# vitskvara/VBMatrixFactorization.jl

Measured on AMD Instinct MI355X. Metric: VB iterations/sec, higher is better.
Workload: dtype bf16

## Files before the change

### vbmatrixfactorization.jl_amd/csrc/gram_kernels.hpp

```cpp
#pragma once
#include "common.hpp"
#include "ctrl_kernels.hpp"
#include "post_kernels.hpp"

namespace vbmf {

#ifndef GRAM_CHUNK
#define GRAM_CHUNK 256
#endif
constexpr int GRAM_PLANES = 5;

__device__ __forceinline__ unsigned pack_bf2(unsigned short lo, unsigned short hi) { return (unsigned)lo | ((unsigned)hi << 16); }

__global__ __launch_bounds__(256) void gram_build_kernel(const uint4* __restrict__ Y1, int XT, int KS, float* __restrict__ Gt,
                                                         int GT) {
    const int P = blockIdx.y, Q = blockIdx.x;
    if (P > Q) return;
    const int lane = threadIdx.x & 63, w = threadIdx.x >> 6;
    const int p0 = 4 * P + 2 * (w >> 1), q0 = 4 * Q + 2 * (w & 1);
    const long long KT = 2LL * GT;
    double g64[2][2][16];
#pragma unroll
    for (int a = 0; a < 2; ++a)
#pragma unroll
// ... 114 lines not shown
            Wnew[m * HP + h] = wv;
            wp[0][e] = f2bf(wv);
            float res = wv - bf2f(wp[0][e]);
            wp[1][e] = f2bf(res);
            res -= bf2f(wp[1][e]);
            wp[2][e] = f2bf(res);
            dp[0][e] = f2bf(dv);
            dp[1][e] = f2bf(dv - bf2f(dp[0][e]));
        }
        const long long o = (j * NH + ht) * 64 + ln;
#pragma unroll
        for (int p = 0; p < 3; ++p)
            Wt[p * plane + o] = make_uint4(pack_bf2(wp[p][0], wp[p][1]), pack_bf2(wp[p][2], wp[p][3]), pack_bf2(wp[p][4], wp[p][5]),
                                           pack_bf2(wp[p][6], wp[p][7]));
#pragma unroll
        for (int p = 0; p < 2; ++p)
            Wt[(3 + p) * plane + o] = make_uint4(pack_bf2(dp[p][0], dp[p][1]), pack_bf2(dp[p][2], dp[p][3]), pack_bf2(dp[p][4], dp[p][5]),
                                                 pack_bf2(dp[p][6], dp[p][7]));
    }
}

__device__ __forceinline__ float sub_f32(float a, float b) {
    float r;
    asm("v_sub_f32 %0, %1, %2" : "=v"(r) : "v"(a), "v"(b));
    return r;
}
__device__ __forceinline__ unsigned cvt_pk_bf16(float lo, float hi) {
    typedef __attribute__((ext_vector_type(2))) float f32x2v;
    typedef __attribute__((ext_vector_type(2))) __bf16 bf16x2v;
    const f32x2v v = {lo, hi};
    return __builtin_bit_cast(unsigned, __builtin_convertvector(v, bf16x2v));
}
__device__ __forceinline__ void split3_frag(const f32x4& x0, const f32x4& x1, u32x4v& g0, u32x4v& g1, u32x4v& g2) {
    const float v[8] = {x0.x, x0.y, x0.z, x0.w, x1.x, x1.y, x1.z, x1.w};
#pragma unroll
    for (int e = 0; e < 4; ++e) {
        float a = v[2 * e], b = v[2 * e + 1];
        const unsigned p0 = cvt_pk_bf16(a, b);
        a = sub_f32(a, bitsf(p0 << 16));
        b = sub_f32(b, bitsf(p0 & 0xffff0000u));
        const unsigned p1 = cvt_pk_bf16(a, b);
        a = sub_f32(a, bitsf(p1 << 16));
        b = sub_f32(b, bitsf(p1 & 0xffff0000u));
        g0[e] = p0;
        g1[e] = p1;
        g2[e] = cvt_pk_bf16(a, b);
    }
}

__device__ __forceinline__ f32x16 mfma_bf(const u32x4v& a, const u32x4v& b, const f32x16& c) {
    return __builtin_amdgcn_mfma_f32_32x32x16_bf16(__builtin_bit_cast(bf16x8, a), __builtin_bit_cast(bf16x8, b), c, 0, 0, 0);
}

template <int NH>
struct GramProd {
    static constexpr int NW = 8;
    static constexpr int THREADS = 64 * NW;
    static constexpr int TPG = 16 / NH;
    static constexpr int NXW = TPG >= NW ? TPG / NW : 1;
    static constexpr int HS = TPG >= NW ? 1 : NW / TPG;
    static constexpr int NHW = NH / HS;
    static constexpr int CH = NH == 2 ? 4 : 2;
    static constexpr int D = 4;
    static constexpr int U = CH;
    static constexpr int NP = GRAM_PLANES * CH * NH;
    static constexpr int PPW = (NP + NW - 1) / NW;
    static constexpr int GL = 2 * NXW;
    static constexpr int PLANE_BYTES = 2 * NP * 1024;
    static constexpr int RING_BYTES = NW * D * GL * 1024;
    static constexpr int LDS_BYTES = PLANE_BYTES + RING_BYTES;
    static_assert(NXW * (NW / HS) == TPG && NHW * HS == NH, "gram_prod geometry");
    static_assert(LDS_BYTES <= 160 * 1024, "gram_prod LDS");
    static constexpr int g_wait(int u) {
        int n = (D - 1) * GL;
        for (int d = 1; d < D; ++d) n += ((u + CH * D - d) % CH == 0) ? PPW : 0;
        return n;
    }
};
template <int NH>
__global__ __launch_bounds__(GramProd<NH>::THREADS) void gram_prod_kernel(const float4* __restrict__ Gt, const uint4* __restrict__ Wt,
                                                                          float* __restrict__ Out, int GT, int XT1, int sps, int nrg,
                                                                          long long n, long long slab_floats,
                                                                          const int* __restrict__ stop) {
    using C = GramProd<NH>;
    constexpr int NW = C::NW, NXW = C::NXW, NHW = C::NHW, D = C::D, CH = C::CH, U = C::U, NP = C::NP, PPW = C::PPW, GL = C::GL;
    extern __shared__ __attribute__((aligned(1024))) unsigned char gram_lds[];
    if (*stop) return;
    const int lane = threadIdx.x & 63;
    const int w = __builtin_amdgcn_readfirstlane(threadIdx.x >> 6);
    const int rg = blockIdx.x % nrg, s = blockIdx.x / nrg;
    const int KT = 2 * GT;
    const int j0 = s * sps, j1 = min(j0 + sps, KT), nk = j1 - j0;
    const int pt0 = rg * C::TPG + (w % (C::TPG / NXW)) * NXW;
    const int h0 = (w / (C::TPG / NXW)) * NHW;
    const long long plane = (long long)KT * NH * 64;
    f32x16 accP[NXW][NHW], accQ[NXW][NHW];
#pragma unroll
    for (int i = 0; i < NXW; ++i)
#pragma unroll
        for (int h = 0; h < NHW; ++h)
#pragma unroll
            for (int r = 0; r < 16; ++r) { accP[i][h][r] = 0.f; accQ[i][h][r] = 0.f; }
    __amdgpu_buffer_rsrc_t gr[NXW];
#pragma unroll
    for (int i = 0; i < NXW; ++i)
        gr[i] = __builtin_amdgcn_make_buffer_rsrc((void*)(Gt + (long long)(pt0 + i) * KT * 128), 0, (unsigned)KT * 2048u, 0x00020000);
    const __amdgpu_buffer_rsrc_t wr = __builtin_amdgcn_make_buffer_rsrc((void*)Wt, 0, (unsigned)(GRAM_PLANES * plane * 16), 0x00020000);
    const int voff = lane * 16;
    unsigned char* const ring = gram_lds + C::PLANE_BYTES + w * (D * GL * 1024);
    auto load_g = [&](int slot, int t) __attribute__((always_inline)) {
        const int so = min(j0 + t, j1 - 1) * 2048;
#pragma unroll
        for (int i = 0; i < NXW; ++i) {
            lds_dma_piece(gr[i], ring + (slot * GL + 2 * i) * 1024, voff, so);
            lds_dma_piece(gr[i], ring + (slot * GL + 2 * i + 1) * 1024, voff, so + 1024);
        }
    };
    auto load_planes = [&](int cc, int t) __attribute__((always_inline)) {
#pragma unroll
        for (int v = 0; v < PPW; ++v) {
            const int x = min(w + NW * v, NP - 1);
            const int q = x / (CH * NH), r = x % (CH * NH);
            const int j = min(j0 + t + r / NH, j1 - 1);
            lds_dma_piece(wr, gram_lds + (cc * NP + x) * 1024, voff, (int)(q * plane + ((long long)j * NH + r % NH) * 64) * 16);
        }
    };
#pragma unroll
    for (int d = 0; d < D; ++d) {
        if ((d + CH * D - D) % CH == 0) load_planes(0, 0);
        load_g(d, d);
    }
    asm volatile("s_waitcnt vmcnt(%0)" ::"n"(CH * GL) : "memory");
    __builtin_amdgcn_s_barrier();
    asm volatile("" ::: "memory");
    u32x4v wf[GRAM_PLANES][NHW], g[NXW][3];
    auto mma = [&]() __attribute__((always_inline)) {
#pragma unroll
        for (int i = 0; i < NXW; ++i) {
#pragma unroll
            for (int h = 0; h < NHW; ++h) {
                f32x16 a = accP[i][h];
                a = mfma_bf(wf[2][h], g[i][0], a);
                a = mfma_bf(wf[1][h], g[i][1], a);
                a = mfma_bf(wf[0][h], g[i][2], a);
                a = mfma_bf(wf[1][h], g[i][0], a);
                a = mfma_bf(wf[0][h], g[i][1], a);
                accP[i][h] = mfma_bf(wf[0][h], g[i][0], a);
                f32x16 d = accQ[i][h];
                d = mfma_bf(wf[4][h], g[i][0], d);
                d = mfma_bf(wf[3][h], g[i][1], d);
                accQ[i][h] = mfma_bf(wf[3][h], g[i][0], d);
            }
        }
    };
    int slot = 0;
    auto body = [&](int t0, bool tail) __attribute__((always_inline)) {
#pragma unroll
        for (int u = 0; u < U; ++u) {
            const int t = t0 + u, kk = u % CH;
            const int cc = (t / CH) & 1;
            const bool live = !tail || t < nk;
            asm volatile("s_waitcnt vmcnt(%0)" ::"n"(C::g_wait(u)) : "memory");
            if (live) {
                const unsigned char* gs = ring + slot * (GL * 1024) + lane * 32;
                f32x4 x[NXW][2];
#pragma unroll
                for (int i = 0; i < NXW; ++i) {
                    x[i][0] = *reinterpret_cast<const f32x4*>(gs + i * 2048);
                    x[i][1] = *reinterpret_cast<const f32x4*>(gs + i * 2048 + 16);
                }
                const unsigned char* pl = gram_lds + (cc * NP + kk * NH + h0) * 1024 + lane * 16;
#pragma unroll
                for (int q = 0; q < GRAM_PLANES; ++q)
#pragma unroll
                    for (int h = 0; h < NHW; ++h) wf[q][h] = *reinterpret_cast<const u32x4v*>(pl + (q * CH * NH + h) * 1024);
#pragma unroll
                for (int i = 0; i < NXW; ++i) split3_frag(x[i][0], x[i][1], g[i][0], g[i][1], g[i][2]);
            }
            __builtin_amdgcn_sched_barrier(0);
            if (kk == 0) load_planes(cc ^ 1, t + CH);
            load_g(slot, t + D);
            slot = slot + 1 == D ? 0 : slot + 1;
            __builtin_amdgcn_sched_barrier(0);
            if (live) mma();
            if (kk == CH - 1) {
                asm volatile("s_waitcnt vmcnt(%0) lgkmcnt(0)" ::"n"(CH * GL) : "memory");
                __builtin_amdgcn_s_barrier();
                asm volatile("" ::: "memory");
            }
        }
    };
    int t0 = 0;
    for (; t0 + U <= nk; t0 += U) body(t0, false);
    if (t0 < nk) body(t0, true);
    asm volatile("s_waitcnt vmcnt(0)" ::: "memory");
    float4* oP = reinterpret_cast<float4*>(Out + (long long)s * slab_floats);
    float4* oQ = reinterpret_cast<float4*>(Out + (long long)s * slab_floats + n);
#pragma unroll
    for (int i = 0; i < NXW; ++i) {
        const int p = pt0 + i;
        if (p >= XT1) continue;
#pragma unroll
        for (int h = 0; h < NHW; ++h) {
            const long long o = (((long long)p * NH + h0 + h) * 64 + lane) * 4;
            const f32x16 a = accP[i][h], d = accQ[i][h];
#pragma unroll
            for (int q = 0; q < 4; ++q) {
                oP[o + q] = float4{a[4 * q], a[4 * q + 1], a[4 * q + 2], a[4 * q + 3]};
                oQ[o + q] = float4{d[4 * q], d[4 * q + 1], d[4 * q + 2], d[4 * q + 3]};
            }
        }
    }
}

template <int HP>
struct GPart {
    static constexpr int V = HP / 16, S = 8 / V, NH = HP / 32;
};
template <int HP>
__device__ __forceinline__ int gpart_index(int a, int b) {
    constexpr int V = GPart<HP>::V;
    const int tw = a % V, i = a / V, t = b % V, c = b / V;
    return ((((tw * V + t) * 4 + (i >> 2)) << 6) + 16 * (i & 3) + c);
}
template <int HP>
__global__ __launch_bounds__(1024) void gram_part_kernel(const float* __restrict__ PQ, long long n, const float* __restrict__ Wn,
                                                         const float* __restrict__ Wo, const float* __restrict__ A32, long long M,
                                                         int rpc, double* __restrict__ part, const int* __restrict__ stop) {
    if (*stop) return;
    constexpr int V = GPart<HP>::V, S = GPart<HP>::S, NH = GPart<HP>::NH, U = 4;
    __shared__ f64x4 fold[S > 1 ? (S - 1) * 2 * V * V * 64 : 1];
    __shared__ double red[16];
    const int lane = threadIdx.x & 63, w = threadIdx.x >> 6;
    const int s = w / (2 * V), task = w % (2 * V), pi = task / V, tw = task % V;
    const int q = lane >> 4, c = lane & 15;
    const float* src = PQ + (pi ? n : 0);
    f64x4 acc[V];
#pragma unroll
    for (int t = 0; t < V; ++t) acc[t] = f64x4{0.0, 0.0, 0.0, 0.0};
    double tr = 0.0;
    const long long m0 = (long long)blockIdx.x * rpc, m1 = min(m0 + rpc, M);
    const int nstep = (int)((m1 - m0 + 3) / 4);
    for (int k0 = s; k0 < nstep; k0 += S * U) {
        float pv[U][V], wv[U], xv[U];
#pragma unroll
        for (int u = 0; u < U; ++u) {
            const long long m = m0 + 4LL * (k0 + u * S) + q;
            if (m < m1) {
                if constexpr (V == 2) {
                    const float2 v = *reinterpret_cast<const float2*>(src + frag_index(2 * c, m, NH));
                    pv[u][0] = v.x; pv[u][1] = v.y;
                } else {
#pragma unroll
                    for (int g = 0; g < V / 4; ++g) {
                        const float4 v = *reinterpret_cast<const float4*>(src + frag_index(V * c + 4 * g, m, NH));
                        pv[u][4 * g] = v.x; pv[u][4 * g + 1] = v.y; pv[u][4 * g + 2] = v.z; pv[u][4 * g + 3] = v.w;
                    }
                }
                wv[u] = Wn[m * HP + V * c + tw];
                xv[u] = (pi ? Wo : A32)[m * HP + V * c + tw];
            } else {
#pragma unroll
                for (int t = 0; t < V; ++t) pv[u][t] = 0.f;
                wv[u] = 0.f; xv[u] = 0.f;
            }
        }
#pragma unroll
        for (int u = 0; u < U; ++u) {
            double a = (double)wv[u];
            if (pi) a = (double)(float)(a - (double)xv[u]);
            else {
                float p = 0.f;
#pragma unroll
                for (int t = 0; t < V; ++t) p = t == tw ? pv[u][t] : p;
                tr += (double)xv[u] * (double)p;
            }
#pragma unroll
            for (int t = 0; t < V; ++t) acc[t] = __builtin_amdgcn_mfma_f64_16x16x4f64(a, (double)pv[u][t], acc[t], 0, 0, 0);
        }
    }
    if constexpr (S > 1) {
        if (s > 0) {
#pragma unroll
            for (int t = 0; t < V; ++t) fold[(((s - 1) * 2 * V + task) * V + t) * 64 + lane] = acc[t];
        }
        __syncthreads();
        if (s == 0) {
            for (int s2 = 1; s2 < S; ++s2)
#pragma unroll
                for (int t = 0; t < V; ++t) acc[t] += fold[(((s2 - 1) * 2 * V + task) * V + t) * 64 + lane];
        }
    }
    double* o = part + (long long)blockIdx.x * (2 * HP * HP + 1) + pi * HP * HP;
    if (s == 0) {
#pragma unroll
        for (int t = 0; t < V; ++t)
#pragma unroll
            for (int r = 0; r < 4; ++r) o[(((tw * V + t) * 4 + r) << 6) + lane] = acc[t][r];
    }
    tr = block_sum(tr, red);
    if (threadIdx.x == 0) part[(long long)blockIdx.x * (2 * HP * HP + 1) + 2 * HP * HP] = tr;
}

constexpr int GRED_E = 64, GRED_G = 4;
template <int HP>
__global__ __launch_bounds__(256) void gram_part_reduce_kernel(const double* __restrict__ part, int nchunk, double* __restrict__ st,
                                                               StateLayout lay, const int* __restrict__ stop) {
    if (*stop) return;
    constexpr int V = GPart<HP>::V, n2 = HP * HP;
    constexpr long long stride = 2LL * n2 + 1;
    __shared__ double sum[2][GRED_G][GRED_E];
    const int el = threadIdx.x % GRED_E, g = threadIdx.x / GRED_E;
    const int e = blockIdx.x * GRED_E + el;
    const int pi = e / n2, x = e % n2;
    const int tw = (x >> 8) / V, t = (x >> 8) % V, rq = (x >> 6) & 3, q = (x >> 4) & 3, c = x & 15;
    const int a = V * (q + 4 * rq) + tw, b = V * c + t;
    const bool mat = e < 2 * n2, tro = e == 2 * n2;
    const long long i0 = mat ? e : 2LL * n2, i1 = mat ? (long long)pi * n2 + gpart_index<HP>(b, a) : 2LL * n2;
    double s0 = 0.0, s1 = 0.0;
    if (mat || tro) {
        int k = g;
        for (; k + 7 * GRED_G < nchunk; k += 8 * GRED_G) {
            double v0[8], v1[8];
#pragma unroll
            for (int u = 0; u < 8; ++u) { v0[u] = part[(k + u * GRED_G) * stride + i0]; v1[u] = part[(k + u * GRED_G) * stride + i1]; }
#pragma unroll
            for (int u = 0; u < 8; ++u) { s0 += v0[u]; s1 += v1[u]; }
        }
        for (; k < nchunk; k += GRED_G) { s0 += part[k * stride + i0]; s1 += part[k * stride + i1]; }
    }
    sum[0][g][el] = s0;
    sum[1][g][el] = s1;
    __syncthreads();
    if (g != 0 || !(mat || tro)) return;
    double t0 = 0.0, t1 = 0.0;
    for (int k = 0; k < GRED_G; ++k) { t0 += sum[0][k][el]; t1 += sum[1][k][el]; }
    if (tro) st[lay.GX()] = t0;
    else st[(pi ? lay.GD() : lay.GB()) + a * HP + b] = 0.5 * (t0 + t1);
}

}
```

### vbmatrixfactorization.jl_amd/csrc/vbmf_hip.hip

```cpp
#include "../../include/vbmf_hip.h"

#include <hip/hip_runtime.h>
#include <rccl/rccl.h>

#include <algorithm>
#include <cmath>
#include <cstdio>
#include <cstring>
#include <string>
#include <vector>

#include "common.hpp"
#include "ctrl_kernels.hpp"
#include "post_kernels.hpp"
#include "rng.hpp"
#include "sparse_kernels.hpp"
#include "stream_gemm.hpp"
#include "tile_kernels.hpp"
#include "prep_kernels.hpp"
#include "batch_kernels.hpp"
#include "sparse_batch_kernels.hpp"
#include "score_kernels.hpp"
#include "gram_kernels.hpp"

// ... 880 lines not shown
        if (e != hipSuccess) {
            for (void* b : {(void*)c->Gt, (void*)c->W32g[0], (void*)c->W32g[1], (void*)c->Wt, (void*)c->gPQ, (void*)c->gslabs,
                            (void*)c->g_part, (void*)c->gsave})
                if (b) hipFree(b);
            c->Gt = nullptr; c->W32g[0] = c->W32g[1] = nullptr; c->Wt = nullptr; c->gPQ = nullptr; c->gslabs = nullptr;
            c->g_part = nullptr; c->gsave = nullptr;
            FAIL(c, VBMF_ERR_HIP, "Gram-form sweep: device allocation failed (%s)", hipGetErrorString(e));
        }
        c->G_valid = false;
    }
    if (c->G_valid) return VBMF_OK;
    hipEvent_t a, b;
    HIPCHK(c, hipEventCreate(&a));
    HIPCHK(c, hipEventCreate(&b));
    hipEventRecord(a, c->stream);
    const int NB = c->GT / 4;
    hipLaunchKernelGGL(gram_build_kernel, dim3(NB, NB), dim3(256), 0, c->stream, c->Y1, c->d1.XT, c->d1.KS, c->Gt, c->GT);
    const hipError_t le = hipGetLastError();
    hipEventRecord(b, c->stream);
    const hipError_t se = hipEventSynchronize(b);
    float ms = 0.f;
    hipEventElapsedTime(&ms, a, b);
    hipEventDestroy(a);
    hipEventDestroy(b);
    HIPCHK(c, le);
    HIPCHK(c, se);
    c->gram_build_ms = ms;
    c->G_valid = true;
    c->W_valid = false;
    return VBMF_OK;
}

static int gram_product(vbmf_ctx* c, bool partials) {
    const int* stop = c->ints + I_STOP;
    const int KT = 2 * c->GT;
    const int64_t Mp1 = (int64_t)c->d1.XT * 32;
    const long long n = (long long)c->Hp * Mp1;
    const float* Wo = c->W32g[c->wcur];
    float* Wn = c->W32g[c->wcur ^ 1];
    const dim3 wg(cdiv(KT, GW_KS));
    if (c->Hp == 32) hipLaunchKernelGGL((gram_w_kernel<32>), wg, dim3(128), 0, c->stream, c->A32, c->SB32, Wo, Wn, c->Wt, (long long)c->M, KT, stop);
    else if (c->Hp == 64) hipLaunchKernelGGL((gram_w_kernel<64>), wg, dim3(256), 0, c->stream, c->A32, c->SB32, Wo, Wn, c->Wt, (long long)c->M, KT, stop);
    else hipLaunchKernelGGL((gram_w_kernel<128>), wg, dim3(512), 0, c->stream, c->A32, c->SB32, Wo, Wn, c->Wt, (long long)c->M, KT, stop);
    HIPCHK(c, hipGetLastError());
    float* out = c->g_nsplit > 1 ? c->gslabs : c->gPQ;
    const dim3 grid(c->g_nrg * c->g_nsplit);
    const float4* G4 = reinterpret_cast<const float4*>(c->Gt);
    prof_begin(c, 0);
    if (c->NH == 1) hipLaunchKernelGGL((gram_prod_kernel<1>), grid, dim3(GramProd<1>::THREADS), GramProd<1>::LDS_BYTES, c->stream, G4, c->Wt, out, c->GT, c->d1.XT, c->g_sps, c->g_nrg, n, 2 * n, stop);
    else if (c->NH == 2) hipLaunchKernelGGL((gram_prod_kernel<2>), grid, dim3(GramProd<2>::THREADS), GramProd<2>::LDS_BYTES, c->stream, G4, c->Wt, out, c->GT, c->d1.XT, c->g_sps, c->g_nrg, n, 2 * n, stop);
    else hipLaunchKernelGGL((gram_prod_kernel<4>), grid, dim3(GramProd<4>::THREADS), GramProd<4>::LDS_BYTES, c->stream, G4, c->Wt, out, c->GT, c->d1.XT, c->g_sps, c->g_nrg, n, 2 * n, stop);
    prof_end(c);
    HIPCHK(c, hipGetLastError());
    if (c->g_nsplit > 1) {
        hipLaunchKernelGGL(slab_sum_kernel, dim3(grid_for(2 * n / 4, 256, 2048)), dim3(256), 0, c->stream, c->gslabs, c->g_nsplit, 2 * n,
                           c->gPQ, 2 * n, stop, SideCopy{});
        HIPCHK(c, hipGetLastError());
    }
    if (partials) {
        const dim3 pg(c->g_nchunk);
        if (c->Hp == 32) hipLaunchKernelGGL((gram_part_kernel<32>), pg, dim3(1024), 0, c->stream, c->gPQ, n, Wn, Wo, c->A32, (long long)c->M, c->g_rpc, c->g_part, stop);
        else if (c->Hp == 64) hipLaunchKernelGGL((gram_part_kernel<64>), pg, dim3(1024), 0, c->stream, c->gPQ, n, Wn, Wo, c->A32, (long long)c->M, c->g_rpc, c->g_part, stop);
        else hipLaunchKernelGGL((gram_part_kernel<128>), pg, dim3(1024), 0, c->stream, c->gPQ, n, Wn, Wo, c->A32, (long long)c->M, c->g_rpc, c->g_part, stop);
        HIPCHK(c, hipGetLastError());
        const dim3 rg(cdiv(2 * (int64_t)c->Hp * c->Hp + 1, GRED_E));
        if (c->Hp == 32) hipLaunchKernelGGL((gram_part_reduce_kernel<32>), rg, dim3(256), 0, c->stream, c->g_part, c->g_nchunk, c->st, c->lay, stop);
        else if (c->Hp == 64) hipLaunchKernelGGL((gram_part_reduce_kernel<64>), rg, dim3(256), 0, c->stream, c->g_part, c->g_nchunk, c->st, c->lay, stop);
        else hipLaunchKernelGGL((gram_part_reduce_kernel<128>), rg, dim3(256), 0, c->stream, c->g_part, c->g_nchunk, c->st, c->lay, stop);
        HIPCHK(c, hipGetLastError());
    }
    return VBMF_OK;
}

template <int R>
static void launch_chain_t(vbmf_ctx* c, const CtrlArgs& ca) {
    hipLaunchKernelGGL((ctrl_chain_kernel<R>), dim3(2), dim3(256), ctrl_lds_bytes_r(R), c->stream, ca);
}
static int launch_chain(vbmf_ctx* c, int mode, float* S32) {
    CtrlArgs ca{};
    ca.st = c->st; ca.lay = c->lay; ca.ints = c->ints; ca.trace = c->run_trace;
    ca.S32 = S32;
    ca.Lg = (double)c->Lg; ca.M = (double)c->M; ca.eps = c->run_eps;
    ca.H = (int)c->H; ca.spectral = spectral_arg(c);
    ca.end_flags = c->run_flags; ca.mode = mode; ca.it_row = (int)c->ends_enqueued;
    const int H = (int)c->H;
    if (H <= 16) launch_chain_t<1>(c, ca);
    else if (H <= 32) launch_chain_t<2>(c, ca);
    else if (H <= 64) launch_chain_t<4>(c, ca);
    else if (H <= 128) launch_chain_t<8>(c, ca);
    else FAIL(c, VBMF_ERR_INVALID, "internal: the stand-alone control chain covers H <= 128");
    HIPCHK(c, hipGetLastError());
    return VBMF_OK;
}

static int gram_sweep(vbmf_ctx* c) {
    TRY(launch_chain(c, CTRL_COV_A | (c->tail_pending ? CTRL_PREV_END : 0), c->SA32));
    if (c->tail_pending) ++c->ends_enqueued;
    c->tail_pending = false;
    c->P_frag = true;
    if (fused_gram(c)) TRY(launch_post_gram(c, 0, c->gPQ));
    else {
        TRY(launch_post_frag(c, 0, c->gPQ));
        TRY(launch_gram(c, 0, c->A32, nullptr, true));
    }
    TRY(launch_chain(c, CTRL_COMMIT_A | CTRL_COV_B | CTRL_EIG_BOLD, c->SB32));
    TRY(gram_product(c, true));
    c->wcur ^= 1;
    c->gA_valid = c->gB_valid = true;
    c->P_valid = false;
    c->tr_valid = true;
    return VBMF_OK;
}

static int prepare_trYBA(vbmf_ctx* c, int* flag) {
    *flag = 0;
    if (c->tr_valid) return VBMF_OK;
// ... 2230 lines not shown
    TRY(ensure_gram_B(c));
    const int H = (int)c->H;
    const int64_t nb = nbags, MH = (int64_t)c->M * H, h2 = (int64_t)H * H;
    const int64_t o_r2 = 2 * (nb + 1), o_part = o_r2 + nb, o_a = o_part + ns, o_ds = o_a + MH, o_ca = o_ds + MH, o_be = o_ca + MH,
                  o_sa = o_be + MH, o_sums = o_sa + nb * h2, o_quad = o_sums + nb * H * SCORE_NS, total = o_quad + 2 * nb;
    TRY(score_reserve(c, total));
    double* d = c->score;
    HIPCHK(c, hipMemcpyAsync(d + o_a, ATVecHat, (size_t)MH * 8, hipMemcpyHostToDevice, c->stream));
    HIPCHK(c, hipMemcpyAsync(d + o_ds, diagSigmaATVec, (size_t)MH * 8, hipMemcpyHostToDevice, c->stream));
    HIPCHK(c, hipMemcpyAsync(d + o_ca, CA, (size_t)MH * 8, hipMemcpyHostToDevice, c->stream));
    HIPCHK(c, hipMemcpyAsync(d + o_be, beta, (size_t)MH * 8, hipMemcpyHostToDevice, c->stream));
    HIPCHK(c, hipMemcpyAsync(d + o_sa, SigmaA, (size_t)(nb * h2) * 8, hipMemcpyHostToDevice, c->stream));
    long long* d_off = reinterpret_cast<long long*>(d);
    TRY(score_launch_resid(c, nb, col_off, ns, d_off, d + o_a, (long long)H, 1, d + o_part, d + o_r2));
    hipLaunchKernelGGL(bag_lb_sums_kernel, dim3((unsigned)nb), dim3(SCORE_THREADS), 0, c->stream, d + o_a, d + o_ds, d + o_ca, d + o_be,
                       d + o_sa, c->st, c->lay, H, (double)c->Lg, d_off, trim, d + o_sums, d + o_quad);
    HIPCHK(c, hipGetLastError());
    std::vector<double> res((size_t)nb), sums((size_t)(total - o_sums)), buf((size_t)c->lay.total());
    HIPCHK(c, hipMemcpyAsync(res.data(), d + o_r2, (size_t)nb * 8, hipMemcpyDeviceToHost, c->stream));
    HIPCHK(c, hipMemcpyAsync(sums.data(), d + o_sums, sums.size() * 8, hipMemcpyDeviceToHost, c->stream));
    HIPCHK(c, memcpy_sync(c, buf.data(), c->st, buf.size() * 8, hipMemcpyDeviceToHost));
    LbSums s{};
    lb_basis_sums(c, buf, s);
    const bool trimmed = trim >= 0.0;
    std::vector<LbGroup> grp((size_t)H);
    const double* quad = sums.data() + (o_quad - o_sums);
    for (int64_t b = 0; b < nb; ++b) {
        const double Mb = (double)(col_off[b + 1] - col_off[b]);
        const double* sb = sums.data() + (size_t)b * H * SCORE_NS;
        double n_keep = 0, s_caq = 0, s_logds = 0;
        for (int h = 0; h < H; ++h) {
            const double* v = sb + (size_t)h * SCORE_NS;
            n_keep += v[2]; s_caq += v[5]; s_logds += v[6];
            const bool cut = trimmed && !grouped;
            grp[(size_t)h] = LbGroup{cut ? v[2] : Mb, cut ? v[3] : v[0], cut ? v[4] : v[1], a_pri[b * H + h], b_pri[b * H + h], a_post[b * H + h]};
        }
        s.M = Mb;
        s.MH = trimmed ? n_keep : Mb * (double)H;
        s.sig = sigmaHat[b]; s.zeta = zeta[b]; s.eta = eta[b];
        s.hyp.eta0 = eta0[b]; s.hyp.zeta0 = zeta0[b];
        s.quad = res[(size_t)b] + s.L * quad[2 * b] + quad[2 * b + 1];
        s.s_caq = s_caq; s.s_logds = s_logds;
        s.g = grp.data(); s.ng = H;
        const double v = lb_assemble(s, clamp);
        if (!std::isfinite(v) || !std::isfinite(s.quad) || !std::isfinite(s_caq) || !std::isfinite(s_logds))
            FAIL(c, VBMF_ERR_NUMERIC, "%s: non-finite sum in bag %lld", fn, (long long)b);
        lb[b] = v;
        if (r2) r2[b] = res[(size_t)b];
    }
    return VBMF_OK;
}

}
```

Measured before the change: 4323.

## Software-pipeline gram_prod: prefetch next k-step operands and interleave bf16 split with MFMAs

Reworks the gram_prod main loop so that the operand registers are double-buffered by k-step parity. The next step's LDS reads happen before the current MFMA chain, and the bf16 three-way split of the next fragment is issued as filler instructions between MFMAs. The P and Q MFMA chains are reordered into six interleaved rounds, and the plane and ring DMA issue points and wait counts are moved, with a compile-time check that the vmcnt waits still cover outstanding loads. It also adds optional s_memtime stamping behind a macro for profiling. The aim is to hide LDS latency and split arithmetic behind matrix-core work, at the cost of more registers, which could lower occupancy or cause spills.

After: 4289. About the same (-0.8%).

```diff
diff --git a/vbmatrixfactorization.jl_amd/csrc/gram_kernels.hpp b/vbmatrixfactorization.jl_amd/csrc/gram_kernels.hpp
--- a/vbmatrixfactorization.jl_amd/csrc/gram_kernels.hpp
+++ b/vbmatrixfactorization.jl_amd/csrc/gram_kernels.hpp
@@ -190,6 +190,18 @@
     return __builtin_amdgcn_mfma_f32_32x32x16_bf16(__builtin_bit_cast(bf16x8, a), __builtin_bit_cast(bf16x8, b), c, 0, 0, 0);
 }
 
+#ifdef GRAM_PROD_STAMP
+constexpr int GRAM_STAMP_SEGS = 6, GRAM_STAMP_WGS = 1024;
+__device__ unsigned long long gram_prod_stamps[GRAM_STAMP_WGS][GRAM_STAMP_SEGS];
+#define GRAM_STAMP(v)                                \
+    do {                                             \
+        __builtin_amdgcn_sched_barrier(0);           \
+        v = __builtin_amdgcn_s_memtime();            \
+        __builtin_amdgcn_sched_barrier(0);           \
+    } while (0)
+#else
+#define GRAM_STAMP(v) do { } while (0)
+#endif
 template <int NH>
 struct GramProd {
     static constexpr int NW = 8;
@@ -209,11 +221,39 @@
     static constexpr int LDS_BYTES = PLANE_BYTES + RING_BYTES;
     static_assert(NXW * (NW / HS) == TPG && NHW * HS == NH, "gram_prod geometry");
     static_assert(LDS_BYTES <= 160 * 1024, "gram_prod LDS");
+    static_assert(U % 2 == 0, "the operand register sets alternate by k-step parity");
+    static constexpr int NA = NXW * NHW;
+    static constexpr int NMMA = 9 * NA;
+    static constexpr int NFILL = 8 * NXW;
+    static constexpr int FILL0 = NFILL + 3 <= NMMA ? 3 : 1;
+    static_assert(FILL0 + NFILL <= NMMA && (3 * NA) % 6 == 0, "one filler behind an MFMA, the Q terms spread evenly over six rounds");
     static constexpr int g_wait(int u) {
         int n = (D - 1) * GL;
-        for (int d = 1; d < D; ++d) n += ((u + CH * D - d) % CH == 0) ? PPW : 0;
+        for (int d = 1; d < D; ++d) n += ((u + CH * D - d) % CH == CH - 1) ? PPW : 0;
         return n;
     }
+    static constexpr int edge_wait(int u) { return g_wait(u) < CH * GL ? g_wait(u) : CH * GL; }
+    static constexpr bool waits_hold() {
+        constexpr int T = 6 * U;
+        int endG[T + D + 1] = {}, endP[T / CH + 3] = {}, n = 0;
+        for (int d = 0; d < D; ++d) {
+            if ((d + CH * D - D) % CH == 0) { n += PPW; endP[0] = n; }
+            n += GL; endG[d] = n;
+        }
+        if (endP[0] > n - edge_wait(CH - 1) || endG[0] > n - edge_wait(CH - 1)) return false;
+        n += PPW; endP[1] = n;
+        n += GL; endG[D] = n;
+        for (int t = 0; t < T; ++t) {
+            const int u = t % U;
+            if (u % CH == CH - 1) {
+                if (endP[t / CH + 1] > n - edge_wait(u) || endG[t + 1] > n - edge_wait(u)) return false;
+                n += PPW; endP[t / CH + 2] = n;
+            } else if (endG[t + 1] > n - g_wait(u)) return false;
+            n += GL; endG[t + 1 + D] = n;
+        }
+        return true;
+    }
+    static_assert(waits_hold(), "gram_prod wait counts");
 };
 template <int NH>
 __global__ __launch_bounds__(GramProd<NH>::THREADS) void gram_prod_kernel(const float4* __restrict__ Gt, const uint4* __restrict__ Wt,
@@ -263,75 +303,138 @@
             lds_dma_piece(wr, gram_lds + (cc * NP + x) * 1024, voff, (int)(q * plane + ((long long)j * NH + r % NH) * 64) * 16);
         }
     };
+    u32x4v wf[2][GRAM_PLANES][NHW], g[2][NXW][3];
+    f32x4 x[NXW][2];
+    int slot = 0;
+#ifdef GRAM_PROD_STAMP
+    unsigned long long seg[4] = {0, 0, 0, 0}, c0, c1, c2, c3, c4;
+    GRAM_STAMP(c0);
+    const unsigned long long cbegin = c0;
+#endif
+    auto read_ahead = [&](int st, int cc, int kk) __attribute__((always_inline)) {
+        const unsigned char* gs = ring + slot * (GL * 1024) + lane * 32;
+#pragma unroll
+        for (int i = 0; i < NXW; ++i) {
+            x[i][0] = *reinterpret_cast<const f32x4*>(gs + i * 2048);
+            x[i][1] = *reinterpret_cast<const f32x4*>(gs + i * 2048 + 16);
+        }
+        __builtin_amdgcn_sched_barrier(0);
+        const unsigned char* pl = gram_lds + (cc * NP + kk * NH + h0) * 1024 + lane * 16;
+#pragma unroll
+        for (int q = 0; q < GRAM_PLANES; ++q)
+#pragma unroll
+            for (int h = 0; h < NHW; ++h) wf[st][q][h] = *reinterpret_cast<const u32x4v*>(pl + (q * CH * NH + h) * 1024);
+    };
+    float ra = 0.f, rb = 0.f;
+    auto filler = [&](int st, int f, int t) __attribute__((always_inline)) {
+        const int i = f / 8, e = (f / 2) % 4;
+        if (f % 8 == 6) {
+            asm volatile("" : "+v"(x[i][0]), "+v"(x[i][1])::"memory");
+            const int so = min(j0 + t + D, j1 - 1) * 2048;
+            lds_dma_piece(gr[i], ring + (slot * GL + 2 * i) * 1024, voff, so);
+            lds_dma_piece(gr[i], ring + (slot * GL + 2 * i + 1) * 1024, voff, so + 1024);
+        }
+        if (f % 2 == 0) {
+            ra = x[i][e >> 1][(2 * e) & 3];
+            rb = x[i][e >> 1][(2 * e + 1) & 3];
+            const unsigned p0 = cvt_pk_bf16(ra, rb);
+            ra = sub_f32(ra, bitsf(p0 << 16));
+            rb = sub_f32(rb, bitsf(p0 & 0xffff0000u));
+            g[st][i][0][e] = p0;
+        } else {
+            const unsigned p1 = cvt_pk_bf16(ra, rb);
+            ra = sub_f32(ra, bitsf(p1 << 16));
+            rb = sub_f32(rb, bitsf(p1 & 0xffff0000u));
+            g[st][i][1][e] = p1;
+            g[st][i][2][e] = cvt_pk_bf16(ra, rb);
+        }
+    };
+    auto mma = [&](int st, bool ahead, int t) __attribute__((always_inline)) {
+        constexpr int PW[6] = {2, 1, 0, 1, 0, 0}, PG[6] = {0, 1, 2, 0, 1, 0}, QW[3] = {4, 3, 3}, QG[3] = {0, 1, 0};
+        int m = 0;
+        auto fill = [&]() __attribute__((always_inline)) {
+            __builtin_amdgcn_sched_barrier(0);
+            const int f = m++ - C::FILL0;
+            if (ahead && f >= 0 && f < C::NFILL) {
+                filler(st ^ 1, f, t + 1);
+                __builtin_amdgcn_sched_barrier(0);
+                if (f == C::NFILL - 1) GRAM_STAMP(c3);
+            }
+        };
+#pragma unroll
+        for (int r = 0; r < 6; ++r) {
+#pragma unroll
+            for (int a = 0; a < C::NA; ++a) {
+                const int i = a / NHW, h = a % NHW;
+                accP[i][h] = mfma_bf(wf[st][PW[r]][h], g[st][i][PG[r]], accP[i][h]);
+                fill();
+            }
+#pragma unroll
+            for (int q = C::NA * r / 2; q < C::NA * (r + 1) / 2; ++q) {
+                const int i = (q % C::NA) / NHW, h = (q % C::NA) % NHW, k = q / C::NA;
+                accQ[i][h] = mfma_bf(wf[st][QW[k]][h], g[st][i][QG[k]], accQ[i][h]);
+                fill();
+            }
+        }
+    };
 #pragma unroll
     for (int d = 0; d < D; ++d) {
         if ((d + CH * D - D) % CH == 0) load_planes(0, 0);
         load_g(d, d);
     }
-    asm volatile("s_waitcnt vmcnt(%0)" ::"n"(CH * GL) : "memory");
+    asm volatile("s_waitcnt vmcnt(%0)" ::"n"(C::edge_wait(CH - 1)) : "memory");
     __builtin_amdgcn_s_barrier();
     asm volatile("" ::: "memory");
-    u32x4v wf[GRAM_PLANES][NHW], g[NXW][3];
-    auto mma = [&]() __attribute__((always_inline)) {
-#pragma unroll
-        for (int i = 0; i < NXW; ++i) {
-#pragma unroll
-            for (int h = 0; h < NHW; ++h) {
-                f32x16 a = accP[i][h];
-                a = mfma_bf(wf[2][h], g[i][0], a);
-                a = mfma_bf(wf[1][h], g[i][1], a);
-                a = mfma_bf(wf[0][h], g[i][2], a);
-                a = mfma_bf(wf[1][h], g[i][0], a);
-                a = mfma_bf(wf[0][h], g[i][1], a);
-                accP[i][h] = mfma_bf(wf[0][h], g[i][0], a);
-                f32x16 d = accQ[i][h];
-                d = mfma_bf(wf[4][h], g[i][0], d);
-                d = mfma_bf(wf[3][h], g[i][1], d);
-                accQ[i][h] = mfma_bf(wf[3][h], g[i][0], d);
-            }
-        }
-    };
-    int slot = 0;
+    load_planes(1, CH);
+    read_ahead(0, 0, 0);
+    __builtin_amdgcn_sched_barrier(0);
+#pragma unroll
+    for (int f = 0; f < C::NFILL; ++f) filler(0, f, 0);
+    slot = 1;
+    GRAM_STAMP(c0);
     auto body = [&](int t0, bool tail) __attribute__((always_inline)) {
 #pragma unroll
         for (int u = 0; u < U; ++u) {
-            const int t = t0 + u, kk = u % CH;
+            const int t = t0 + u, kk = u % CH, st = u & 1;
             const int cc = (t / CH) & 1;
-            const bool live = !tail || t < nk;
-            asm volatile("s_waitcnt vmcnt(%0)" ::"n"(C::g_wait(u)) : "memory");
-            if (live) {
-                const unsigned char* gs = ring + slot * (GL * 1024) + lane * 32;
-                f32x4 x[NXW][2];
-#pragma unroll
-                for (int i = 0; i < NXW; ++i) {
-                    x[i][0] = *reinterpret_cast<const f32x4*>(gs + i * 2048);
-                    x[i][1] = *reinterpret_cast<const f32x4*>(gs + i * 2048 + 16);
-                }
-                const unsigned char* pl = gram_lds + (cc * NP + kk * NH + h0) * 1024 + lane * 16;
-#pragma unroll
-                for (int q = 0; q < GRAM_PLANES; ++q)
-#pragma unroll
-                    for (int h = 0; h < NHW; ++h) wf[q][h] = *reinterpret_cast<const u32x4v*>(pl + (q * CH * NH + h) * 1024);
-#pragma unroll
-                for (int i = 0; i < NXW; ++i) split3_frag(x[i][0], x[i][1], g[i][0], g[i][1], g[i][2]);
-            }
-            __builtin_amdgcn_sched_barrier(0);
-            if (kk == 0) load_planes(cc ^ 1, t + CH);
-            load_g(slot, t + D);
-            slot = slot + 1 == D ? 0 : slot + 1;
-            __builtin_amdgcn_sched_barrier(0);
-            if (live) mma();
+            const bool live = !tail || t < nk, ahead = !tail || t + 1 < nk;
             if (kk == CH - 1) {
-                asm volatile("s_waitcnt vmcnt(%0) lgkmcnt(0)" ::"n"(CH * GL) : "memory");
+                asm volatile("s_waitcnt vmcnt(%0) lgkmcnt(0)" ::"n"(C::edge_wait(u)) : "memory");
                 __builtin_amdgcn_s_barrier();
                 asm volatile("" ::: "memory");
-            }
+                load_planes(cc, t + 1 + CH);
+            } else {
+                asm volatile("s_waitcnt vmcnt(%0)" ::"n"(C::g_wait(u)) : "memory");
+            }
+            GRAM_STAMP(c1);
+            if (ahead) read_ahead(st ^ 1, kk == CH - 1 ? cc ^ 1 : cc, (kk + 1) % CH);
+            else load_g(slot, t + 1 + D);
+            __builtin_amdgcn_sched_barrier(0);
+            GRAM_STAMP(c2);
+#ifdef GRAM_PROD_STAMP
+            c3 = c2;
+#endif
+            if (live) mma(st, ahead, t);
+            __builtin_amdgcn_sched_barrier(0);
+#ifdef GRAM_PROD_STAMP
+            GRAM_STAMP(c4);
+            seg[0] += c1 - c0; seg[1] += c2 - c1; seg[2] += c3 - c2; seg[3] += c4 - c3;
+            c0 = c4;
+#endif
+            slot = slot + 1 == D ? 0 : slot + 1;
         }
     };
     int t0 = 0;
     for (; t0 + U <= nk; t0 += U) body(t0, false);
     if (t0 < nk) body(t0, true);
     asm volatile("s_waitcnt vmcnt(0)" ::: "memory");
+#ifdef GRAM_PROD_STAMP
+    if (threadIdx.x == 0 && blockIdx.x < GRAM_STAMP_WGS) {
+        for (int k = 0; k < 4; ++k) gram_prod_stamps[blockIdx.x][k] = seg[k];
+        gram_prod_stamps[blockIdx.x][4] = c0 - cbegin;
+        gram_prod_stamps[blockIdx.x][5] = (unsigned long long)nk;
+    }
+#endif
     float4* oP = reinterpret_cast<float4*>(Out + (long long)s * slab_floats);
     float4* oQ = reinterpret_cast<float4*>(Out + (long long)s * slab_floats + n);
 #pragma unroll
diff --git a/vbmatrixfactorization.jl_amd/csrc/vbmf_hip.hip b/vbmatrixfactorization.jl_amd/csrc/vbmf_hip.hip
--- a/vbmatrixfactorization.jl_amd/csrc/vbmf_hip.hip
+++ b/vbmatrixfactorization.jl_amd/csrc/vbmf_hip.hip
@@ -3302,3 +3302,10 @@
 }
 
 }
+
+#ifdef GRAM_PROD_STAMP
+extern "C" int vbmf_debug_gram_stamps(unsigned long long* out, int nwg) {
+    if (nwg < 0 || nwg > vbmf::GRAM_STAMP_WGS) return -1;
+    return (int)hipMemcpyFromSymbol(out, HIP_SYMBOL(vbmf::gram_prod_stamps), sizeof(unsigned long long) * vbmf::GRAM_STAMP_SEGS * (size_t)nwg);
+}
+#endif
```

## Fuse slab summation into gram partials kernel with LDS-staged double buffering

Applied to the files above, without the earlier changes.

Replaces the separate slab_sum kernel and gram_part kernel with one gram_tail kernel. Each block sums the split slabs for its row chunk, writes the summed P/Q back, and stages the rows in LDS for the f64 MFMA partial products. It double-buffers across row blocks and prefetches W and X with buffer loads. The partial reduce is also restructured into fixed-depth rounds with clamped loads. This removes one kernel launch and the global round-trip of the summed slabs, at the cost of more register pressure and more complex indexing.

New measurement: 4309 before, 4376 after (median of 6 runs). 1.6% higher.

```diff
diff --git a/vbmatrixfactorization.jl_amd/csrc/gram_kernels.hpp b/vbmatrixfactorization.jl_amd/csrc/gram_kernels.hpp
--- a/vbmatrixfactorization.jl_amd/csrc/gram_kernels.hpp
+++ b/vbmatrixfactorization.jl_amd/csrc/gram_kernels.hpp
@@ -354,6 +354,14 @@
 template <int HP>
 struct GPart {
     static constexpr int V = HP / 16, S = 8 / V, NH = HP / 32;
+    static constexpr int NT = 512, SD = 8;
+    static constexpr int PPT = HP == 128 ? 2 : 3;
+    static constexpr int ROWS = PPT * NT * 4 / HP;
+    static constexpr int NSTEP = ROWS / 4 / S;
+    static constexpr int BUF = ROWS * HP;
+    static constexpr int SU = V == 8 ? 2 : 4;
+    static_assert(NSTEP % SU == 0 && (ROWS / 4) % S == 0 && ROWS % 16 == 0, "gram_tail geometry");
+    static_assert((S - 1) * V * V * 64 * 32 <= 2 * BUF * 4, "gram_tail: the subset fold reuses the block buffers");
 };
 template <int HP>
 __device__ __forceinline__ int gpart_index(int a, int b) {
@@ -361,90 +369,220 @@
     const int tw = a % V, i = a / V, t = b % V, c = b / V;
     return ((((tw * V + t) * 4 + (i >> 2)) << 6) + 16 * (i & 3) + c);
 }
+__device__ __forceinline__ void add4(float4& s, const float4& v) { s.x += v.x; s.y += v.y; s.z += v.z; s.w += v.w; }
+struct GTailRound { float4 a0, a1, a2, a3, a4, a5, a6, a7; };
+__device__ __forceinline__ void gtail_load(GTailRound& v, const __amdgpu_buffer_rsrc_t (&r)[8], int voff, int cnt) {
+    const auto ld = [&](int u) __attribute__((always_inline)) {
+        return __builtin_bit_cast(float4, __builtin_amdgcn_raw_buffer_load_b128(r[u], voff, 0, 0));
+    };
+    switch (cnt) {
+        default: v.a7 = ld(7); [[fallthrough]];
+        case 7: v.a6 = ld(6); [[fallthrough]];
+        case 6: v.a5 = ld(5); [[fallthrough]];
+        case 5: v.a4 = ld(4); [[fallthrough]];
+        case 4: v.a3 = ld(3); [[fallthrough]];
+        case 3: v.a2 = ld(2); [[fallthrough]];
+        case 2: v.a1 = ld(1); [[fallthrough]];
+        case 1: v.a0 = ld(0);
+    }
+}
+template <bool FIRST>
+__device__ __forceinline__ float4 gtail_sum(const GTailRound& v, float4 f, int cnt) {
+    if (FIRST) f = v.a0;
+    else add4(f, v.a0);
+    if (cnt > 1) add4(f, v.a1);
+    if (cnt > 2) add4(f, v.a2);
+    if (cnt > 3) add4(f, v.a3);
+    if (cnt > 4) add4(f, v.a4);
+    if (cnt > 5) add4(f, v.a5);
+    if (cnt > 6) add4(f, v.a6);
+    if (cnt > 7) add4(f, v.a7);
+    return f;
+}
 template <int HP>
-__global__ __launch_bounds__(1024) void gram_part_kernel(const float* __restrict__ PQ, long long n, const float* __restrict__ Wn,
-                                                         const float* __restrict__ Wo, const float* __restrict__ A32, long long M,
-                                                         int rpc, double* __restrict__ part, const int* __restrict__ stop) {
-    if (*stop) return;
-    constexpr int V = GPart<HP>::V, S = GPart<HP>::S, NH = GPart<HP>::NH, U = 4;
-    __shared__ f64x4 fold[S > 1 ? (S - 1) * 2 * V * V * 64 : 1];
-    __shared__ double red[16];
-    const int lane = threadIdx.x & 63, w = threadIdx.x >> 6;
-    const int s = w / (2 * V), task = w % (2 * V), pi = task / V, tw = task % V;
+__global__ __launch_bounds__(512) void gram_tail_kernel(const float* slabs, int nslab, long long slab_floats, float* PQ, long long n,
+                                                        long long Mp1, const float* __restrict__ Wn, const float* __restrict__ Wo,
+                                                        const float* __restrict__ A32, long long M, int rpc, int nchunk,
+                                                        double* __restrict__ part, const int* __restrict__ stop) {
+    using C = GPart<HP>;
+    constexpr int V = C::V, S = C::S, NH = C::NH, PPT = C::PPT, SD = C::SD, ROWS = C::ROWS, NSTEP = C::NSTEP, SU = C::SU;
+    __shared__ __attribute__((aligned(32))) float stage[2 * C::BUF];
+    __shared__ double red[8];
+    const int stopv = *stop;
+    const int lane = threadIdx.x & 63;
+    const int w = __builtin_amdgcn_readfirstlane(threadIdx.x >> 6);
+    const int s = w / V, tw = w % V;
     const int q = lane >> 4, c = lane & 15;
-    const float* src = PQ + (pi ? n : 0);
+    const int chunk = blockIdx.x >> 1, pi = blockIdx.x & 1;
+    const long long m0 = (long long)chunk * rpc, m1 = min(m0 + rpc, M);
+    const long long fend = chunk == nchunk - 1 ? Mp1 : m0 + rpc;
+    const float* src = slabs + (pi ? n : 0);
+    float* dst = PQ + (pi ? n : 0);
+    const float* X = pi ? Wo : A32;
+    const int xr = lane >> 2, r4 = lane & 3;
+    int grp[PPT], ht[PPT], half[PPT];
+#pragma unroll
+    for (int j = 0; j < PPT; ++j) {
+        const int sg = 8 * j + w;
+        grp[j] = sg / (2 * NH);
+        ht[j] = (sg % (2 * NH)) >> 1;
+        half[j] = sg & 1;
+    }
+    GTailRound v[PPT];
+    static_assert(SD == 8, "gram_tail: GTailRound");
+    float wv[NSTEP], xv[NSTEP];
+    auto piece_off = [&](long long rb, int j) __attribute__((always_inline)) {
+        const long long row = rb + 16 * grp[j] + xr;
+        return ((((row >> 5) * NH + ht[j]) * 64 + half[j] * 32 + (row & 31)) << 4) + 4 * r4;
+    };
+    auto issue_slabs = [&](long long rb, int k0) __attribute__((always_inline)) {
+        __amdgpu_buffer_rsrc_t r[SD];
+#pragma unroll
+        for (int u = 0; u < SD; ++u)
+            r[u] = __builtin_amdgcn_make_buffer_rsrc((void*)(src + (long long)(k0 + u) * slab_floats), 0, (unsigned)(n * 4), 0x00020000);
+#pragma unroll
+        for (int j = 0; j < PPT; ++j) {
+            if (rb + 16 * grp[j] >= fend) continue;
+            gtail_load(v[j], r, (int)(piece_off(rb, j) * 4), min(SD, nslab - k0));
+        }
+    };
+    auto fold_slabs = [&](long long rb, int k0, float4 (&f)[PPT]) __attribute__((always_inline)) {
+#pragma unroll
+        for (int j = 0; j < PPT; ++j) {
+            if (rb + 16 * grp[j] >= fend) continue;
+            if (k0 == 0) f[j] = gtail_sum<true>(v[j], f[j], min(SD, nslab));
+            else f[j] = gtail_sum<false>(v[j], f[j], min(SD, nslab - k0));
+        }
+    };
+    const __amdgpu_buffer_rsrc_t wr = __builtin_amdgcn_make_buffer_rsrc((void*)Wn, 0, (unsigned)(m1 * HP * 4), 0x00020000);
+    const __amdgpu_buffer_rsrc_t xd = __builtin_amdgcn_make_buffer_rsrc((void*)X, 0, (unsigned)(m1 * HP * 4), 0x00020000);
+    auto issue_w = [&](long long rb) __attribute__((always_inline)) {
+        const int o = (int)(((rb + 4 * s + q) * HP + V * c + tw) * 4);
+#pragma unroll
+        for (int i = 0; i < NSTEP; ++i) {
+            wv[i] = bitsf(__builtin_amdgcn_raw_buffer_load_b32(wr, o + i * (4 * S * HP * 4), 0, 0));
+            xv[i] = bitsf(__builtin_amdgcn_raw_buffer_load_b32(xd, o + i * (4 * S * HP * 4), 0, 0));
+        }
+    };
+    issue_slabs(m0, 0);
+    issue_w(m0);
+    if (stopv) return;
     f64x4 acc[V];
 #pragma unroll
     for (int t = 0; t < V; ++t) acc[t] = f64x4{0.0, 0.0, 0.0, 0.0};
     double tr = 0.0;
-    const long long m0 = (long long)blockIdx.x * rpc, m1 = min(m0 + rpc, M);
-    const int nstep = (int)((m1 - m0 + 3) / 4);
-    for (int k0 = s; k0 < nstep; k0 += S * U) {
-        float pv[U][V], wv[U], xv[U];
-#pragma unroll
-        for (int u = 0; u < U; ++u) {
-            const long long m = m0 + 4LL * (k0 + u * S) + q;
-            if (m < m1) {
+    int buf = 0;
+    for (long long rb = m0; rb < fend; rb += ROWS, buf ^= 1) {
+        float* sb = stage + buf * C::BUF;
+        float4 f[PPT];
+        fold_slabs(rb, 0, f);
+        for (int k0 = SD; k0 < nslab; k0 += SD) {
+            issue_slabs(rb, k0);
+            fold_slabs(rb, k0, f);
+        }
+#pragma unroll
+        for (int j = 0; j < PPT; ++j) {
+            if (rb + 16 * grp[j] >= fend) continue;
+            if (nslab > 1) *reinterpret_cast<float4*>(dst + piece_off(rb, j)) = f[j];
+            *reinterpret_cast<float4*>(sb + (16 * grp[j] + xr) * HP + 32 * ht[j] + 8 * r4 + 4 * half[j]) = f[j];
+        }
+        float ac[NSTEP], xc[NSTEP];
+#pragma unroll
+        for (int i = 0; i < NSTEP; ++i) {
+            xc[i] = xv[i];
+            ac[i] = pi ? (float)((double)wv[i] - (double)xc[i]) : wv[i];
+        }
+        if (rb + ROWS < fend) {
+            issue_slabs(rb + ROWS, 0);
+            issue_w(rb + ROWS);
+        }
+        asm volatile("s_waitcnt lgkmcnt(0)" ::: "memory");
+        __builtin_amdgcn_s_barrier();
+        asm volatile("" ::: "memory");
+#pragma unroll
+        for (int i0 = 0; i0 < NSTEP; i0 += SU) {
+            if (rb + 4 * (s + S * i0) >= m1) break;
+            __builtin_amdgcn_sched_barrier(0);
+#pragma unroll
+            for (int i = i0; i < i0 + SU; ++i) {
+                const int rl = 4 * (s + S * i) + q;
+                const bool in = rb + rl < m1;
+                float pv[V];
                 if constexpr (V == 2) {
-                    const float2 v = *reinterpret_cast<const float2*>(src + frag_index(2 * c, m, NH));
-                    pv[u][0] = v.x; pv[u][1] = v.y;
+                    const float2 x = *reinterpret_cast<const float2*>(sb + rl * HP + 2 * c);
+                    pv[0] = x.x; pv[1] = x.y;
                 } else {
 #pragma unroll
                     for (int g = 0; g < V / 4; ++g) {
-                        const float4 v = *reinterpret_cast<const float4*>(src + frag_index(V * c + 4 * g, m, NH));
-                        pv[u][4 * g] = v.x; pv[u][4 * g + 1] = v.y; pv[u][4 * g + 2] = v.z; pv[u][4 * g + 3] = v.w;
+                        const float4 x = *reinterpret_cast<const float4*>(sb + rl * HP + V * c + 4 * g);
+                        pv[4 * g] = x.x; pv[4 * g + 1] = x.y; pv[4 * g + 2] = x.z; pv[4 * g + 3] = x.w;
                     }
                 }
-                wv[u] = Wn[m * HP + V * c + tw];
-                xv[u] = (pi ? Wo : A32)[m * HP + V * c + tw];
-            } else {
-#pragma unroll
-                for (int t = 0; t < V; ++t) pv[u][t] = 0.f;
-                wv[u] = 0.f; xv[u] = 0.f;
+#pragma unroll
+                for (int t = 0; t < V; ++t) pv[t] = in ? pv[t] : 0.f;
+                if (!pi) {
+                    float p = 0.f;
+#pragma unroll
+                    for (int t = 0; t < V; ++t) p = t == tw ? pv[t] : p;
+                    tr += (double)xc[i] * (double)p;
+                }
+#pragma unroll
+                for (int t = 0; t < V; ++t) acc[t] = __builtin_amdgcn_mfma_f64_16x16x4f64((double)ac[i], (double)pv[t], acc[t], 0, 0, 0);
             }
         }
-#pragma unroll
-        for (int u = 0; u < U; ++u) {
-            double a = (double)wv[u];
-            if (pi) a = (double)(float)(a - (double)xv[u]);
-            else {
-                float p = 0.f;
-#pragma unroll
-                for (int t = 0; t < V; ++t) p = t == tw ? pv[u][t] : p;
-                tr += (double)xv[u] * (double)p;
-            }
-#pragma unroll
-            for (int t = 0; t < V; ++t) acc[t] = __builtin_amdgcn_mfma_f64_16x16x4f64(a, (double)pv[u][t], acc[t], 0, 0, 0);
-        }
     }
     if constexpr (S > 1) {
+        f64x4* fold = reinterpret_cast<f64x4*>(stage);
+        __syncthreads();
         if (s > 0) {
 #pragma unroll
-            for (int t = 0; t < V; ++t) fold[(((s - 1) * 2 * V + task) * V + t) * 64 + lane] = acc[t];
+            for (int t = 0; t < V; ++t) fold[(((s - 1) * V + tw) * V + t) * 64 + lane] = acc[t];
         }
         __syncthreads();
         if (s == 0) {
             for (int s2 = 1; s2 < S; ++s2)
 #pragma unroll
-                for (int t = 0; t < V; ++t) acc[t] += fold[(((s2 - 1) * 2 * V + task) * V + t) * 64 + lane];
-        }
-    }
-    double* o = part + (long long)blockIdx.x * (2 * HP * HP + 1) + pi * HP * HP;
+                for (int t = 0; t < V; ++t) acc[t] += fold[(((s2 - 1) * V + tw) * V + t) * 64 + lane];
+        }
+    }
+    double* o = part + (long long)chunk * (2 * HP * HP + 1) + pi * HP * HP;
     if (s == 0) {
 #pragma unroll
         for (int t = 0; t < V; ++t)
 #pragma unroll
             for (int r = 0; r < 4; ++r) o[(((tw * V + t) * 4 + r) << 6) + lane] = acc[t][r];
     }
-    tr = block_sum(tr, red);
-    if (threadIdx.x == 0) part[(long long)blockIdx.x * (2 * HP * HP + 1) + 2 * HP * HP] = tr;
+    if (pi) return;
+    for (int off = 32; off > 0; off >>= 1) tr += __shfl_down(tr, off);
+    if (lane == 0) red[w] = tr;
+    __syncthreads();
+    if (threadIdx.x == 0) {
+        double t = 0.0;
+        for (int i = 0; i < 8; ++i) t += red[i];
+        part[(long long)chunk * (2 * HP * HP + 1) + 2 * HP * HP] = t;
+    }
 }
 
 constexpr int GRED_E = 64, GRED_G = 4;
+template <int DP>
+__device__ __forceinline__ void gred_round(const double* __restrict__ part, int k, int nchunk, long long stride, long long i0,
+                                           long long i1, double& s0, double& s1) {
+    double v0[DP], v1[DP];
+#pragma unroll
+    for (int u = 0; u < DP; ++u) {
+        const long long o = (long long)min(k + u * GRED_G, nchunk - 1) * stride;
+        v0[u] = part[o + i0];
+        v1[u] = part[o + i1];
+    }
+    __builtin_amdgcn_sched_barrier(0);
+#pragma unroll
+    for (int u = 0; u < DP; ++u)
+        if (k + u * GRED_G < nchunk) { s0 += v0[u]; s1 += v1[u]; }
+}
 template <int HP>
 __global__ __launch_bounds__(256) void gram_part_reduce_kernel(const double* __restrict__ part, int nchunk, double* __restrict__ st,
                                                                StateLayout lay, const int* __restrict__ stop) {
-    if (*stop) return;
+    const int stopv = *stop;
     constexpr int V = GPart<HP>::V, n2 = HP * HP;
     constexpr long long stride = 2LL * n2 + 1;
     __shared__ double sum[2][GRED_G][GRED_E];
@@ -456,17 +594,13 @@
     const bool mat = e < 2 * n2, tro = e == 2 * n2;
     const long long i0 = mat ? e : 2LL * n2, i1 = mat ? (long long)pi * n2 + gpart_index<HP>(b, a) : 2LL * n2;
     double s0 = 0.0, s1 = 0.0;
-    if (mat || tro) {
-        int k = g;
-        for (; k + 7 * GRED_G < nchunk; k += 8 * GRED_G) {
-            double v0[8], v1[8];
-#pragma unroll
-            for (int u = 0; u < 8; ++u) { v0[u] = part[(k + u * GRED_G) * stride + i0]; v1[u] = part[(k + u * GRED_G) * stride + i1]; }
-#pragma unroll
-            for (int u = 0; u < 8; ++u) { s0 += v0[u]; s1 += v1[u]; }
-        }
-        for (; k < nchunk; k += GRED_G) { s0 += part[k * stride + i0]; s1 += part[k * stride + i1]; }
-    }
+    for (int k = g; k < nchunk; k += 32 * GRED_G) {
+        const int left = (nchunk - k + GRED_G - 1) / GRED_G;
+        if (left <= 8) gred_round<8>(part, k, nchunk, stride, i0, i1, s0, s1);
+        else if (left <= 16) gred_round<16>(part, k, nchunk, stride, i0, i1, s0, s1);
+        else gred_round<32>(part, k, nchunk, stride, i0, i1, s0, s1);
+    }
+    if (stopv) return;
     sum[0][g][el] = s0;
     sum[1][g][el] = s1;
     __syncthreads();
diff --git a/vbmatrixfactorization.jl_amd/csrc/vbmf_hip.hip b/vbmatrixfactorization.jl_amd/csrc/vbmf_hip.hip
--- a/vbmatrixfactorization.jl_amd/csrc/vbmf_hip.hip
+++ b/vbmatrixfactorization.jl_amd/csrc/vbmf_hip.hip
@@ -956,16 +956,18 @@
     else hipLaunchKernelGGL((gram_prod_kernel<4>), grid, dim3(GramProd<4>::THREADS), GramProd<4>::LDS_BYTES, c->stream, G4, c->Wt, out, c->GT, c->d1.XT, c->g_sps, c->g_nrg, n, 2 * n, stop);
     prof_end(c);
     HIPCHK(c, hipGetLastError());
-    if (c->g_nsplit > 1) {
-        hipLaunchKernelGGL(slab_sum_kernel, dim3(grid_for(2 * n / 4, 256, 2048)), dim3(256), 0, c->stream, c->gslabs, c->g_nsplit, 2 * n,
-                           c->gPQ, 2 * n, stop, SideCopy{});
-        HIPCHK(c, hipGetLastError());
-    }
-    if (partials) {
-        const dim3 pg(c->g_nchunk);
-        if (c->Hp == 32) hipLaunchKernelGGL((gram_part_kernel<32>), pg, dim3(1024), 0, c->stream, c->gPQ, n, Wn, Wo, c->A32, (long long)c->M, c->g_rpc, c->g_part, stop);
-        else if (c->Hp == 64) hipLaunchKernelGGL((gram_part_kernel<64>), pg, dim3(1024), 0, c->stream, c->gPQ, n, Wn, Wo, c->A32, (long long)c->M, c->g_rpc, c->g_part, stop);
-        else hipLaunchKernelGGL((gram_part_kernel<128>), pg, dim3(1024), 0, c->stream, c->gPQ, n, Wn, Wo, c->A32, (long long)c->M, c->g_rpc, c->g_part, stop);
+    if (!partials) {
+        if (c->g_nsplit > 1) {
+            hipLaunchKernelGGL(slab_sum_kernel, dim3(grid_for(2 * n / 4, 256, 2048)), dim3(256), 0, c->stream, c->gslabs, c->g_nsplit, 2 * n,
+                               c->gPQ, 2 * n, stop, SideCopy{});
+            HIPCHK(c, hipGetLastError());
+        }
+    } else {
+        const dim3 tg(2 * c->g_nchunk);
+        const long long M = (long long)c->M;
+        if (c->Hp == 32) hipLaunchKernelGGL((gram_tail_kernel<32>), tg, dim3(512), 0, c->stream, out, c->g_nsplit, 2 * n, c->gPQ, n, (long long)Mp1, Wn, Wo, c->A32, M, c->g_rpc, c->g_nchunk, c->g_part, stop);
+        else if (c->Hp == 64) hipLaunchKernelGGL((gram_tail_kernel<64>), tg, dim3(512), 0, c->stream, out, c->g_nsplit, 2 * n, c->gPQ, n, (long long)Mp1, Wn, Wo, c->A32, M, c->g_rpc, c->g_nchunk, c->g_part, stop);
+        else hipLaunchKernelGGL((gram_tail_kernel<128>), tg, dim3(512), 0, c->stream, out, c->g_nsplit, 2 * n, c->gPQ, n, (long long)Mp1, Wn, Wo, c->A32, M, c->g_rpc, c->g_nchunk, c->g_part, stop);
         HIPCHK(c, hipGetLastError());
         const dim3 rg(cdiv(2 * (int64_t)c->Hp * c->Hp + 1, GRED_E));
         if (c->Hp == 32) hipLaunchKernelGGL((gram_part_reduce_kernel<32>), rg, dim3(256), 0, c->stream, c->g_part, c->g_nchunk, c->st, c->lay, stop);
```
